# PersiaML/PERSIA

Hardware: AMD Instinct MI355X
Metric: samples/sec (whole node), DLRM-style hybrid training (higher is better)
Workload: dtype bf16; 1 GPU; preset=criteo, model=dlrm 26sparse/13dense dim128, global_batch=8192, rows=100000000, capacity_per_rank=100000000, staleness=8, parallelism=dp1+emb-a2a

## Files before the change

persia_amd/csrc/interact.hip:

```cpp
#include <torch/extension.h>
#include <ATen/hip/HIPContext.h>
#include <hip/hip_runtime.h>
#include <hip/hip_bf16.h>

namespace {

using bf16x8i = __attribute__((ext_vector_type(8))) short;
using bf16x4i = __attribute__((__vector_size__(4 * sizeof(__bf16)))) __bf16;
using f32x4i = __attribute__((ext_vector_type(4))) float;

__device__ __forceinline__ float ibf2f(short x) {
  union { float f; unsigned u; } v;
  v.u = ((unsigned)(unsigned short)x) << 16;
  return v.f;
}

__device__ __forceinline__ short if2bf(float f) {
  union { float f; unsigned u; } v;
  v.f = f;
  unsigned lsb = (v.u >> 16) & 1;
  v.u += 0x7fff + lsb;
  return (short)(v.u >> 16);
}

constexpr int ceil16(int x) { return (x + 15) & ~15; }
constexpr int ceil32(int x) { return (x + 31) & ~31; }

__global__ __launch_bounds__(256) void interact_fwd_mfma_kernel(
    const short* __restrict__ V, short* __restrict__ out, int B, int F, int D,
    int P) {
  extern __shared__ short lds[];
  const int waves = blockDim.x / 64;
  const int wave = threadIdx.x / 64, lane = threadIdx.x % 64;
  const int Fp = ceil16(F), Dk = ceil32(D);
  const int LDK = Dk + 8;
  const int T = Fp / 16;
  short* v = lds + wave * Fp * LDK;
  for (int t = lane; t < Fp * LDK / 8; t += 64) *(bf16x8i*)&v[t * 8] = bf16x8i{};
  const int fi = lane & 15;
  const int fk8 = (lane >> 4) * 8;
  const int d8 = D / 8;
  for (int64_t b = (int64_t)blockIdx.x * waves + wave; b < B;
       b += (int64_t)gridDim.x * waves) {
    const short* src = V + b * F * D;
    for (int t = lane; t < F * d8; t += 64) {
      const int fr = t / d8, c8 = (t % d8) * 8;
      *(bf16x8i*)&v[fr * LDK + c8] = *(const bf16x8i*)&src[fr * D + c8];
    }
    short* dst = out + b * P;
    for (int ti = 0; ti < T; ++ti) {
      for (int tj = 0; tj <= ti; ++tj) {
        f32x4i acc = {};
        for (int k = 0; k < Dk; k += 32) {
          const bf16x8i a = *(const bf16x8i*)&v[(ti * 16 + fi) * LDK + k + fk8];
          const bf16x8i c = *(const bf16x8i*)&v[(tj * 16 + fi) * LDK + k + fk8];
          acc = __builtin_amdgcn_mfma_f32_16x16x32_bf16(a, c, acc, 0, 0, 0);
        }
        const int j = tj * 16 + fi;
#pragma unroll
        for (int r = 0; r < 4; ++r) {
          const int i = ti * 16 + (lane >> 4) * 4 + r;
          if (i < F && j < i) dst[i * (i - 1) / 2 + j] = if2bf(acc[r]);
        }
      }
    }
  }
}

__global__ __launch_bounds__(256) void interact_bwd_mfma_kernel(
    const short* __restrict__ g, const short* __restrict__ V,
    short* __restrict__ dV, int B, int F, int D, int P) {
  extern __shared__ short lds[];
  const int waves = blockDim.x / 64;
  const int wave = threadIdx.x / 64, lane = threadIdx.x % 64;
  const int Fp = ceil16(F), Fk = ceil32(F), Dp = ceil16(D);
  const int LDA = Fk + 8;
  short* A = lds + wave * (Fp + Dp) * LDA;
  short* vt = A + Fp * LDA;
  for (int t = lane; t < (Fp + Dp) * LDA / 8; t += 64)
    *(bf16x8i*)&A[t * 8] = bf16x8i{};
  const int Tm = Fp / 16, Tn = Dp / 16;
  const int fi = lane & 15;
  const int fk8 = (lane >> 4) * 8;
  const int d8 = D / 8;
  for (int64_t b = (int64_t)blockIdx.x * waves + wave; b < B;
       b += (int64_t)gridDim.x * waves) {
    const short* src = V + b * F * D;
    for (int t = lane; t < F * d8; t += 64) {
      const int fr = t / d8, c8 = (t % d8) * 8;
      const bf16x8i row = *(const bf16x8i*)&src[fr * D + c8];
#pragma unroll
      for (int k = 0; k < 8; ++k) vt[(c8 + k) * LDA + fr] = row[k];
    }
    const short* gp = g + b * P;
    for (int p = lane; p < P; p += 64) {
      int i = (int)((1.0f + sqrtf(1.0f + 8.0f * (float)p)) * 0.5f);
      while (i * (i - 1) / 2 > p) --i;
      while ((i + 1) * i / 2 <= p) ++i;
      const int j = p - i * (i - 1) / 2;
      const short gv = gp[p];
      A[i * LDA + j] = gv;
      A[j * LDA + i] = gv;
    }
    short* dst = dV + b * F * D;
    for (int ti = 0; ti < Tm; ++ti) {
      for (int td = 0; td < Tn; ++td) {
        f32x4i acc = {};
        for (int k = 0; k < Fk; k += 32) {
          const bf16x8i a = *(const bf16x8i*)&A[(ti * 16 + fi) * LDA + k + fk8];
          const bf16x8i c = *(const bf16x8i*)&vt[(td * 16 + fi) * LDA + k + fk8];
          acc = __builtin_amdgcn_mfma_f32_16x16x32_bf16(a, c, acc, 0, 0, 0);
        }
        const int d = td * 16 + fi;
        if (d < D) {
#pragma unroll
          for (int r = 0; r < 4; ++r) {
            const int i = ti * 16 + (lane >> 4) * 4 + r;
            if (i < F) dst[i * D + d] = if2bf(acc[r]);
          }
        }
      }
    }
  }
}

__global__ __launch_bounds__(256) void interact_fwd_packed_kernel(
    const short* __restrict__ x, const __half* __restrict__ base,
    short* __restrict__ out, int B, int S, int D, int P) {
  extern __shared__ short lds[];
  const int F = S + 1;
  const int waves = blockDim.x / 64;
  const int wave = threadIdx.x / 64, lane = threadIdx.x % 64;
  const int Fp = ceil16(F), Dk = ceil32(D);
  const int LDK = Dk + 8;
  const int T = Fp / 16;
  short* v = lds + wave * Fp * LDK;
  for (int t = lane; t < Fp * LDK / 8; t += 64) *(bf16x8i*)&v[t * 8] = bf16x8i{};
  const int fi = lane & 15;
  const int fk8 = (lane >> 4) * 8;
  const int d8 = D / 8;
  for (int64_t b = (int64_t)blockIdx.x * waves + wave; b < B;
       b += (int64_t)gridDim.x * waves) {
    for (int t = lane; t < F * d8; t += 64) {
      const int fr = t / d8, c8 = (t % d8) * 8;
      bf16x8i val;
      if (fr == 0) {
        val = *(const bf16x8i*)&x[b * D + c8];
      } else {
        const __half* src = base + ((int64_t)(fr - 1) * B + b) * D + c8;
#pragma unroll
        for (int k = 0; k < 8; ++k) val[k] = if2bf(__half2float(src[k]));
      }
      *(bf16x8i*)&v[fr * LDK + c8] = val;
    }
    short* dst = out + b * P;
    for (int ti = 0; ti < T; ++ti) {
      for (int tj = 0; tj <= ti; ++tj) {
        f32x4i acc = {};
        for (int k = 0; k < Dk; k += 32) {
          const bf16x8i a = *(const bf16x8i*)&v[(ti * 16 + fi) * LDK + k + fk8];
          const bf16x8i c = *(const bf16x8i*)&v[(tj * 16 + fi) * LDK + k + fk8];
          acc = __builtin_amdgcn_mfma_f32_16x16x32_bf16(a, c, acc, 0, 0, 0);
        }
        const int j = tj * 16 + fi;
#pragma unroll
        for (int r = 0; r < 4; ++r) {
          const int i = ti * 16 + (lane >> 4) * 4 + r;
          if (i < F && j < i) dst[i * (i - 1) / 2 + j] = if2bf(acc[r]);
        }
      }
    }
  }
}

__global__ __launch_bounds__(256) void interact_bwd_packed_kernel(
    const short* __restrict__ g, const short* __restrict__ x,
    const __half* __restrict__ base, short* __restrict__ dx,
    __half* __restrict__ dbase, int B, int S, int D, int P) {
  extern __shared__ short lds[];
  const int F = S + 1;
  const int waves = blockDim.x / 64;
  const int wave = threadIdx.x / 64, lane = threadIdx.x % 64;
  const int Fp = ceil16(F), Fk = ceil32(F), Dp = ceil16(D);
  const int LDA = Fk + 8;
  const int LDV = Dp + 8;
  short* A = lds + wave * (Fp * LDA + Fk * LDV);
  short* v = A + Fp * LDA;
  for (int t = lane; t < (Fp * LDA + Fk * LDV) / 8; t += 64)
    *(bf16x8i*)&A[t * 8] = bf16x8i{};
  const int Tm = Fp / 16, Tn = Dp / 16;
  const int fi = lane & 15;
  const int fk8 = (lane >> 4) * 8;
  const int d8 = D / 8;
  const int t_ro = ((lane & 15) >> 2);
  const int t_co = (lane & 3) * 4;
  auto vtr = [&](int kb, int td) {
    const short* b0 = &v[(kb + fk8 + t_ro) * LDV + td * 16 + t_co];
    bf16x4i lo = __builtin_amdgcn_ds_read_tr16_b64_v4bf16(
        (__attribute__((address_space(3))) bf16x4i*)(void*)const_cast<short*>(b0));
    bf16x4i hi = __builtin_amdgcn_ds_read_tr16_b64_v4bf16(
        (__attribute__((address_space(3))) bf16x4i*)(void*)const_cast<short*>(b0 + 4 * LDV));
    bf16x8i r;
#pragma unroll
    for (int j = 0; j < 4; ++j) {
      r[j] = ((const short*)&lo)[j];
      r[4 + j] = ((const short*)&hi)[j];
    }
    return r;
  };
  for (int64_t b = (int64_t)blockIdx.x * waves + wave; b < B;
       b += (int64_t)gridDim.x * waves) {
    for (int t = lane; t < F * d8; t += 64) {
      const int fr = t / d8, c8 = (t % d8) * 8;
      bf16x8i row;
      if (fr == 0) {
        row = *(const bf16x8i*)&x[b * D + c8];
      } else {
        const __half* src = base + ((int64_t)(fr - 1) * B + b) * D + c8;
#pragma unroll
        for (int k = 0; k < 8; ++k) row[k] = if2bf(__half2float(src[k]));
      }
      *(bf16x8i*)&v[fr * LDV + c8] = row;
    }
    const short* gp = g + b * P;
    for (int p = lane; p < P; p += 64) {
      int i = (int)((1.0f + sqrtf(1.0f + 8.0f * (float)p)) * 0.5f);
      while (i * (i - 1) / 2 > p) --i;
      while ((i + 1) * i / 2 <= p) ++i;
      const int j = p - i * (i - 1) / 2;
      const short gv = gp[p];
      A[i * LDA + j] = gv;
      A[j * LDA + i] = gv;
    }
    for (int ti = 0; ti < Tm; ++ti) {
      for (int td = 0; td < Tn; ++td) {
        f32x4i acc = {};
        for (int k = 0; k < Fk; k += 32) {
          const bf16x8i a = *(const bf16x8i*)&A[(ti * 16 + fi) * LDA + k + fk8];
          const bf16x8i c = vtr(k, td);
          acc = __builtin_amdgcn_mfma_f32_16x16x32_bf16(a, c, acc, 0, 0, 0);
        }
        const int d = td * 16 + fi;
        if (d < D) {
#pragma unroll
          for (int r = 0; r < 4; ++r) {
            const int i = ti * 16 + (lane >> 4) * 4 + r;
            if (i == 0) {
              dx[b * D + d] = if2bf(acc[r]);
            } else if (i < F) {
              dbase[((int64_t)(i - 1) * B + b) * D + d] = __float2half(acc[r]);
            }
          }
        }
      }
    }
  }
}

__global__ __launch_bounds__(256) void interact_fwd_kernel(
    const short* __restrict__ V, short* __restrict__ out, int B, int F, int D,
    int P) {
  extern __shared__ short lds[];
  const int wave = threadIdx.x / 64, lane = threadIdx.x % 64;
  const int LD = D + 8;
  short* v = lds + wave * F * LD;
  const int64_t stride = (int64_t)gridDim.x * 4;
  const int64_t rounds = ((int64_t)B + stride - 1) / stride;
  for (int64_t r = 0; r < rounds; ++r) {
    const int64_t b = r * stride + (int64_t)blockIdx.x * 4 + wave;
    if (b < B) {
      const short* src = V + b * F * D;
      const int d8 = D / 8;
      for (int t = lane; t < F * d8; t += 64) {
        const int fr = t / d8, c8 = (t % d8) * 8;
        *(bf16x8i*)&v[fr * LD + c8] = *(const bf16x8i*)&src[fr * D + c8];
      }
    }
    __syncthreads();
    if (b < B) {
      for (int p = lane; p < P; p += 64) {
        int i = (int)((1.0f + sqrtf(1.0f + 8.0f * (float)p)) * 0.5f);
        while (i * (i - 1) / 2 > p) --i;
        while ((i + 1) * i / 2 <= p) ++i;
        const int j = p - i * (i - 1) / 2;
        const short* vi = &v[i * LD];
        const short* vj = &v[j * LD];
        float acc = 0.0f;
        for (int d = 0; d < D; d += 8) {
          bf16x8i a = *(const bf16x8i*)&vi[d];
          bf16x8i c = *(const bf16x8i*)&vj[d];
#pragma unroll
          for (int k = 0; k < 8; ++k) acc += ibf2f(a[k]) * ibf2f(c[k]);
        }
        out[b * P + p] = if2bf(acc);
      }
    }
    __syncthreads();
  }
}

__global__ __launch_bounds__(256) void interact_bwd_kernel(
    const short* __restrict__ g, const short* __restrict__ V,
    short* __restrict__ dV, int B, int F, int D, int P) {
  extern __shared__ short lds[];
  const int wave = threadIdx.x / 64, lane = threadIdx.x % 64;
  const int LD = D + 8;
  short* v = lds + wave * (F * LD + F * F);
  short* G = v + F * LD;
  const int64_t stride = (int64_t)gridDim.x * 4;
  const int64_t rounds = ((int64_t)B + stride - 1) / stride;
  for (int64_t r = 0; r < rounds; ++r) {
    const int64_t b = r * stride + (int64_t)blockIdx.x * 4 + wave;
    if (b < B) {
      const short* src = V + b * F * D;
      const int d8l = D / 8;
      for (int t = lane; t < F * d8l; t += 64) {
        const int fr = t / d8l, c8 = (t % d8l) * 8;
        *(bf16x8i*)&v[fr * LD + c8] = *(const bf16x8i*)&src[fr * D + c8];
      }
      for (int t = lane; t < F * F; t += 64) G[t] = 0;
    }
    __syncthreads();
    if (b < B) {
      const short* gp = g + b * P;
      for (int p = lane; p < P; p += 64) {
        int i = (int)((1.0f + sqrtf(1.0f + 8.0f * (float)p)) * 0.5f);
        while (i * (i - 1) / 2 > p) --i;
        while ((i + 1) * i / 2 <= p) ++i;
        const int j = p - i * (i - 1) / 2;
        const short gv = gp[p];
        G[i * F + j] = gv;
        G[j * F + i] = gv;
      }
    }
    __syncthreads();
    if (b < B) {
      const int d8 = D / 8;
      short* dst = dV + b * F * D;
      for (int t = lane; t < F * d8; t += 64) {
        const int i = t / d8, dd = (t % d8) * 8;
        float acc[8] = {};
        for (int j = 0; j < F; ++j) {
          const float gij = ibf2f(G[i * F + j]);
          if (gij != 0.0f) {
            const short* vj = &v[j * LD + dd];
#pragma unroll
            for (int k = 0; k < 8; ++k) acc[k] += gij * ibf2f(vj[k]);
          }
        }
#pragma unroll
        for (int k = 0; k < 8; ++k) dst[i * D + dd + k] = if2bf(acc[k]);
      }
    }
    __syncthreads();
  }
}

inline int pick_waves(int per_wave_shorts) {
  const int bytes = per_wave_shorts * 2;
  for (int w = 4; w >= 1; w >>= 1)
    if (w * bytes <= 65536) return w;
  return 0;
}

}

static hipStream_t icur_stream() {
  return at::hip::getCurrentHIPStream().stream();
}

torch::Tensor interact_fwd(torch::Tensor V) {
  TORCH_CHECK(V.scalar_type() == torch::kBFloat16 && V.is_contiguous());
  const int B = (int)V.size(0), F = (int)V.size(1), D = (int)V.size(2);
  TORCH_CHECK(D % 8 == 0);
  const int P = F * (F - 1) / 2;
  auto out = torch::empty(
      {B, P}, torch::TensorOptions().dtype(torch::kBFloat16).device(V.device()));
  const int Fp = ceil16(F), Dk = ceil32(D);
  const int mfma_shorts = Fp * (Dk + 8);
  const int waves = pick_waves(mfma_shorts);
  if (waves > 0) {
    const int grid = std::min((B + waves - 1) / waves, 8192);
    hipLaunchKernelGGL(interact_fwd_mfma_kernel, dim3(grid),
                       dim3(waves * 64), waves * mfma_shorts * 2,
                       icur_stream(), (const short*)V.data_ptr(),
                       (short*)out.data_ptr(), B, F, D, P);
    return out;
  }
  const int lds = 4 * F * (D + 8) * 2;
  TORCH_CHECK(lds <= 65536, "interaction tile exceeds LDS");
  const int grid = std::min((B + 3) / 4, 8192);
  hipLaunchKernelGGL(interact_fwd_kernel, dim3(grid), dim3(256), lds,
                     icur_stream(), (const short*)V.data_ptr(),
                     (short*)out.data_ptr(), B, F, D, P);
  return out;
}

torch::Tensor interact_bwd(torch::Tensor g, torch::Tensor V) {
  const int B = (int)V.size(0), F = (int)V.size(1), D = (int)V.size(2);
  const int P = F * (F - 1) / 2;
  auto dV = torch::empty_like(V);
  const int Fp = ceil16(F), Fk = ceil32(F), Dp = ceil16(D);
  const int mfma_shorts = (Fp + Dp) * (Fk + 8);
  const int waves = pick_waves(mfma_shorts);
  if (waves > 0) {
    const int grid = std::min((B + waves - 1) / waves, 8192);
    hipLaunchKernelGGL(interact_bwd_mfma_kernel, dim3(grid),
                       dim3(waves * 64), waves * mfma_shorts * 2,
                       icur_stream(), (const short*)g.data_ptr(),
                       (const short*)V.data_ptr(), (short*)dV.data_ptr(), B, F,
                       D, P);
    return dV;
  }
  const int lds = 4 * (F * (D + 8) * 2 + 2 * F * F);
  TORCH_CHECK(lds <= 65536, "interaction tile exceeds LDS");
  const int grid = std::min((B + 3) / 4, 8192);
  hipLaunchKernelGGL(interact_bwd_kernel, dim3(grid), dim3(256), lds,
                     icur_stream(), (const short*)g.data_ptr(),
                     (const short*)V.data_ptr(), (short*)dV.data_ptr(), B, F,
                     D, P);
  return dV;
}

torch::Tensor interact_fwd_packed(torch::Tensor x, torch::Tensor base) {
  TORCH_CHECK(x.scalar_type() == torch::kBFloat16 && x.is_contiguous());
  TORCH_CHECK(base.scalar_type() == torch::kFloat16 && base.is_contiguous());
  const int B = (int)x.size(0), D = (int)x.size(1);
  const int S = (int)(base.size(0) / B);
  const int F = S + 1;
  TORCH_CHECK(D % 8 == 0 && base.size(1) == D && base.size(0) == (int64_t)S * B);
  const int P = F * (F - 1) / 2;
  auto out = torch::empty(
      {B, P}, torch::TensorOptions().dtype(torch::kBFloat16).device(x.device()));
  const int Fp = ceil16(F), Dk = ceil32(D);
  const int mfma_shorts = Fp * (Dk + 8);
  const int waves = pick_waves(mfma_shorts);
  TORCH_CHECK(waves > 0, "interact_fwd_packed: tile exceeds LDS");
  const int grid = std::min((B + waves - 1) / waves, 8192);
  hipLaunchKernelGGL(interact_fwd_packed_kernel, dim3(grid), dim3(waves * 64),
                     waves * mfma_shorts * 2, icur_stream(),
                     (const short*)x.data_ptr(),
                     (const __half*)base.data_ptr<at::Half>(),
                     (short*)out.data_ptr(), B, S, D, P);
  return out;
}

std::vector<torch::Tensor> interact_bwd_packed(torch::Tensor g, torch::Tensor x,
                                               torch::Tensor base) {
  const int B = (int)x.size(0), D = (int)x.size(1);
  const int S = (int)(base.size(0) / B);
  const int F = S + 1;
  const int P = F * (F - 1) / 2;
  auto dx = torch::empty_like(x);
  auto dbase = torch::empty_like(base);
  const int Fp = ceil16(F), Fk = ceil32(F), Dp = ceil16(D);
  const int mfma_shorts = Fp * (Fk + 8) + Fk * (Dp + 8);
  const int waves = pick_waves(mfma_shorts);
  TORCH_CHECK(waves > 0, "interact_bwd_packed: tile exceeds LDS");
  const int grid = std::min((B + waves - 1) / waves, 8192);
  auto gc = g.contiguous();
  hipLaunchKernelGGL(interact_bwd_packed_kernel, dim3(grid), dim3(waves * 64),
                     waves * mfma_shorts * 2, icur_stream(),
                     (const short*)gc.data_ptr(),
                     (const short*)x.data_ptr(),
                     (const __half*)base.data_ptr<at::Half>(),
                     (short*)dx.data_ptr(), (__half*)dbase.data_ptr<at::Half>(),
                     B, S, D, P);
  return {dx, dbase};
}

bool interact_packed_feasible(int64_t F, int64_t D) {
  if (D % 8 != 0) return false;
  const int Fp = ceil16((int)F), Fk = ceil32((int)F), Dp = ceil16((int)D),
            Dk = ceil32((int)D);
  return pick_waves(Fp * (Dk + 8)) > 0 &&
         pick_waves(Fp * (Fk + 8) + Fk * (Dp + 8)) > 0;
}

bool interact_feasible(int64_t F, int64_t D) {
  if (D % 8 != 0) return false;
  const int Fp = ceil16((int)F), Fk = ceil32((int)F), Dp = ceil16((int)D),
            Dk = ceil32((int)D);
  const bool fwd_ok = pick_waves(Fp * (Dk + 8)) > 0 ||
                      4 * (int)F * ((int)D + 8) * 2 <= 65536;
  const bool bwd_ok =
      pick_waves((Fp + Dp) * (Fk + 8)) > 0 ||
      4 * ((int)F * ((int)D + 8) * 2 + 2 * (int)F * (int)F) <= 65536;
  return fwd_ok && bwd_ok;
}

void init_interact(pybind11::module_& m) {
  m.def("interact_fwd", &interact_fwd, "DLRM pairwise dot interaction");
  m.def("interact_bwd", &interact_bwd, "interaction backward (dV)");
  m.def("interact_feasible", &interact_feasible,
        "true if a fused interaction kernel exists for (F, D)");
  m.def("interact_packed_feasible", &interact_packed_feasible,
        "true if the packed-input MFMA interaction fits (F, D)");
  m.def("interact_fwd_packed", &interact_fwd_packed,
        "interaction from (x bf16 [B,D], slot-major f16 base) directly");
  m.def("interact_bwd_packed", &interact_bwd_packed,
        "packed interaction backward -> (dx, dbase f16)");
}
```

persia_amd/models/dlrm.py:

```python
from typing import List

import torch
import torch.nn as nn


class _BlasLinearFn(torch.autograd.Function):

    @staticmethod
    def forward(ctx, x, w, b):
        ctx.save_for_backward(x, w)
        return torch.nn.functional.linear(x, w, b)

    @staticmethod
    def backward(ctx, g):
        from persia_amd.ops import native

        x, w = ctx.saved_tensors
        g = g.contiguous()
        dx = g @ w
        dw = g.t() @ x
        db = native().bias_grad(g).to(w.dtype)
        return dx, dw, db


class PALinear(nn.Linear):

    def forward(self, x):
        import os

        if (
            x.is_cuda and x.dim() == 2 and self.bias is not None
            and x.dtype == self.weight.dtype and x.dtype == torch.bfloat16
            and os.environ.get("PA_BLAS_LINEAR", "0") == "1"
        ):
            from persia_amd.ops import native_available

            if native_available():
                return _BlasLinearFn.apply(x, self.weight, self.bias)
        return super().forward(x)


def _mlp(sizes: List[int], last_relu: bool = False) -> nn.Sequential:
    layers: List[nn.Module] = []
    for i in range(len(sizes) - 1):
        layers.append(PALinear(sizes[i], sizes[i + 1]))
        if i < len(sizes) - 2 or last_relu:
            layers.append(nn.ReLU())
    return nn.Sequential(*layers)


class _InteractFn(torch.autograd.Function):

    @staticmethod
    def forward(ctx, v):
        from persia_amd.ops import native

        v = v.to(torch.bfloat16).contiguous()
        ctx.save_for_backward(v)
        return native().interact_fwd(v)

    @staticmethod
    def backward(ctx, g):
        from persia_amd.ops import native

        (v,) = ctx.saved_tensors
        return native().interact_bwd(g.to(torch.bfloat16).contiguous(), v)


class _InteractPackedFn(torch.autograd.Function):

    @staticmethod
    def forward(ctx, x, base):
        from persia_amd.ops import native

        x = x.contiguous()
        base = base.contiguous()
        ctx.save_for_backward(x, base)
        return native().interact_fwd_packed(x, base)

    @staticmethod
    def backward(ctx, g):
        from persia_amd.ops import native

        x, base = ctx.saved_tensors
        dx, dbase = native().interact_bwd_packed(g, x, base)
        return dx, dbase


class DotInteraction(nn.Module):

    def forward(self, vectors: torch.Tensor) -> torch.Tensor:
        F, D = vectors.shape[1], vectors.shape[2]
        if vectors.is_cuda and D % 8 == 0:
            from persia_amd.ops import native, native_available

            if native_available() and native().interact_feasible(F, D):
                return _InteractFn.apply(vectors)
        B, F, _D = vectors.shape
        prod = torch.bmm(vectors, vectors.transpose(1, 2))
        li, lj = torch.tril_indices(F, F, offset=-1, device=vectors.device)
        return prod[:, li, lj]


class DLRM(nn.Module):
    def __init__(
        self,
        num_sparse: int = 26,
        num_dense: int = 13,
        dim: int = 128,
        bottom_mlp: List[int] = (512, 256, 128),
        top_mlp: List[int] = (1024, 1024, 512, 256),
        fused: bool = False,
    ):
        super().__init__()
        self.dim = dim
        self.num_sparse = num_sparse
        n_f = num_sparse + 1
        inter_out = n_f * (n_f - 1) // 2
        if fused:
            from persia_amd.ops.dense import FusedMLP

            self.bottom = FusedMLP([num_dense] + list(bottom_mlp) + [dim], last_relu=True)
            self.top = FusedMLP([dim + inter_out] + list(top_mlp) + [1])
        else:
            self.bottom = _mlp([num_dense] + list(bottom_mlp) + [dim], last_relu=True)
            self.top = _mlp([dim + inter_out] + list(top_mlp) + [1])
        self.interaction = DotInteraction()

    def forward(
        self, non_id_tensors, embedding_tensors
    ) -> torch.Tensor:
        dense = (
            non_id_tensors if torch.is_tensor(non_id_tensors) else non_id_tensors[0]
        )
        dt = next(self.bottom.parameters()).dtype
        dense = dense.to(dt)
        x = self.bottom(dense)
        if torch.is_tensor(embedding_tensors):
            B = x.shape[0]
            if (
                x.is_cuda
                and x.dtype == torch.bfloat16
                and embedding_tensors.dtype == torch.float16
                and self.dim % 8 == 0
            ):
                from persia_amd.ops import native, native_available

                if native_available() and native().interact_packed_feasible(
                    self.num_sparse + 1, self.dim
                ):
                    inter = _InteractPackedFn.apply(x, embedding_tensors)
                    k = x.shape[1] + inter.shape[1]
                    pad = (-k) % 128
                    parts = [x, inter]
                    if pad:
                        parts.append(x.new_zeros(B, pad))
                    return self.top(torch.cat(parts, dim=1)).squeeze(1)
            emb = (
                embedding_tensors.view(self.num_sparse, B, self.dim)
                .permute(1, 0, 2)
                .to(x.dtype)
            )
            vectors = torch.cat([x.unsqueeze(1), emb], dim=1)
        else:
            vectors = torch.stack([x] + [e.to(x.dtype) for e in embedding_tensors], dim=1)
        inter = self.interaction(vectors)
        out = self.top(torch.cat([x, inter], dim=1))
        return out.squeeze(1)
```

Baseline: 7.854 million samples/s.

## Fuse interaction output concat/pad and backward grad slicing into packed kernels

Forward now writes x, the pairwise dot products and the zero padding directly into the padded top-MLP input buffer, which removes the separate torch.cat and zero-fill. A new backward kernel reads the full top-input gradient with a stride, adds the dx slice in-kernel, and can accumulate the embedding gradient in place into base.grad. It also uses vectorized f16->bf16 conversion and the LDS transpose-read instruction (ds_read_tr16) for the dV matmul. This cuts extra elementwise kernels and memory traffic, at the cost of more kernel complexity and a sqrt-based pair index decode per element.

```diff
diff --git a/persia_amd/csrc/interact.hip b/persia_amd/csrc/interact.hip
--- a/persia_amd/csrc/interact.hip
+++ b/persia_amd/csrc/interact.hip
@@ -124,9 +124,10 @@
   }
 }
 
+template <bool INTO>
 __global__ __launch_bounds__(256) void interact_fwd_packed_kernel(
     const short* __restrict__ x, const __half* __restrict__ base,
-    short* __restrict__ out, int B, int S, int D, int P) {
+    short* __restrict__ out, int B, int S, int D, int P, int ldo) {
   extern __shared__ short lds[];
   const int F = S + 1;
   const int waves = blockDim.x / 64;
@@ -146,6 +147,7 @@
       bf16x8i val;
       if (fr == 0) {
         val = *(const bf16x8i*)&x[b * D + c8];
+        if (INTO) *(bf16x8i*)&out[b * ldo + c8] = val;
       } else {
         const __half* src = base + ((int64_t)(fr - 1) * B + b) * D + c8;
 #pragma unroll
@@ -153,7 +155,9 @@
       }
       *(bf16x8i*)&v[fr * LDK + c8] = val;
     }
-    short* dst = out + b * P;
+    short* dst = out + b * ldo + (INTO ? D : 0);
+    if (INTO)
+      for (int t = P + lane; t < ldo - D; t += 64) dst[t] = 0;
     for (int ti = 0; ti < T; ++ti) {
       for (int tj = 0; tj <= ti; ++tj) {
         f32x4i acc = {};
@@ -257,6 +261,179 @@
   }
 }
 
+__device__ __forceinline__ void wave_lds_fence() {
+  asm volatile("s_waitcnt lgkmcnt(0)" ::: "memory");
+  __builtin_amdgcn_wave_barrier();
+}
+
+__device__ __forceinline__ short if2bf_nan(float f) {
+  return f != f ? (short)0x7fc0 : if2bf(f);
+}
+
+using f16x8 = __attribute__((ext_vector_type(8))) _Float16;
+using f16x4 = __attribute__((ext_vector_type(4))) _Float16;
+using f32x8 = __attribute__((ext_vector_type(8))) float;
+using hbf16x8 = __attribute__((ext_vector_type(8))) __bf16;
+using hbf16x4 = __attribute__((ext_vector_type(4))) __bf16;
+using s16x4 = __attribute__((ext_vector_type(4))) short;
+
+__device__ __forceinline__ bf16x8i f16x8_to_bf16(f16x8 h) {
+  const hbf16x8 r =
+      __builtin_convertvector(__builtin_convertvector(h, f32x8), hbf16x8);
+  return __builtin_bit_cast(bf16x8i, r);
+}
+
+struct ChunkWalk {
+  int fr, c;
+  __device__ __forceinline__ void next(int q64, int r64, int d8) {
+    fr += q64;
+    c += r64;
+    if (c >= d8) {
+      c -= d8;
+      ++fr;
+    }
+  }
+};
+
+template <int NK>
+__global__ __launch_bounds__(256) void interact_bwd_packed_io_kernel(
+    const short* __restrict__ g, int ldg, int gcol,
+    const short* __restrict__ x, const __half* __restrict__ base,
+    const short* __restrict__ gx, short* __restrict__ dx, short* dbase,
+    int accumulate, int B, int S, int D, int P) {
+  extern __shared__ short lds[];
+  const int F = S + 1;
+  const int waves = blockDim.x / 64;
+  const int wave = threadIdx.x / 64, lane = threadIdx.x % 64;
+  constexpr int Fk = NK * 32;
+  const int Fp = ceil16(F), Dp = ceil16(D);
+  const int LDA = Fk + 8;
+  const int LDV = Dp + 8;
+  short* A = lds + wave * (Fp * LDA + Fk * LDV);
+  short* v = A + Fp * LDA;
+  for (int t = lane; t < (Fp * LDA + Fk * LDV) / 8; t += 64)
+    *(bf16x8i*)&A[t * 8] = bf16x8i{};
+  const int Tm = Fp / 16, Tn = Dp / 16;
+  const int fi = lane & 15;
+  const int fk8 = (lane >> 4) * 8;
+  const int d8 = D / 8;
+  const int n8 = F * d8;
+  const int t_ro = ((lane & 15) >> 2);
+  const int t_co = (lane & 3) * 4;
+  auto vtr = [&](int kb, int td) {
+    const short* b0 = &v[(kb + fk8 + t_ro) * LDV + td * 16 + t_co];
+    bf16x4i lo = __builtin_amdgcn_ds_read_tr16_b64_v4bf16(
+        (__attribute__((address_space(3))) bf16x4i*)(void*)const_cast<short*>(b0));
+    bf16x4i hi = __builtin_amdgcn_ds_read_tr16_b64_v4bf16(
+        (__attribute__((address_space(3))) bf16x4i*)(void*)const_cast<short*>(b0 + 4 * LDV));
+    bf16x8i r;
+#pragma unroll
+    for (int j = 0; j < 4; ++j) {
+      r[j] = ((const short*)&lo)[j];
+      r[4 + j] = ((const short*)&hi)[j];
+    }
+    return r;
+  };
+  const ChunkWalk w0 = {lane / d8, lane % d8};
+  const int q64 = 64 / d8, r64 = 64 % d8;
+  wave_lds_fence();
+  for (int64_t b = (int64_t)blockIdx.x * waves + wave; b < B;
+       b += (int64_t)gridDim.x * waves) {
+    ChunkWalk w = w0;
+    for (int t = lane; t < n8; t += 64, w.next(q64, r64, d8)) {
+      const int fr = w.fr, c8 = w.c * 8;
+      bf16x8i row;
+      if (fr == 0) {
+        row = *(const bf16x8i*)&x[b * D + c8];
+      } else {
+        row = f16x8_to_bf16(
+            *(const f16x8*)(base + ((int64_t)(fr - 1) * B + b) * D + c8));
+      }
+      *(bf16x8i*)&v[fr * LDV + c8] = row;
+    }
+    const short* gp = g + b * ldg + gcol;
+    for (int p = lane; p < P; p += 64) {
+      int i = (int)((1.0f + sqrtf(1.0f + 8.0f * (float)p)) * 0.5f);
+      while (i * (i - 1) / 2 > p) --i;
+      while ((i + 1) * i / 2 <= p) ++i;
+      const int j = p - i * (i - 1) / 2;
+      const short gv = gp[p];
+      A[i * LDA + j] = gv;
+      A[j * LDA + i] = gv;
+    }
+    wave_lds_fence();
+    for (int td = 0; td < Tn; ++td) {
+      bf16x8i c[NK];
+#pragma unroll
+      for (int kk = 0; kk < NK; ++kk) c[kk] = vtr(kk * 32, td);
+      wave_lds_fence();
+      const int d0 = td * 16 + (lane >> 4) * 4;
+      for (int ti = 0; ti < Tm; ++ti) {
+        f32x4i acc = {};
+#pragma unroll
+        for (int kk = 0; kk < NK; ++kk) {
+          const bf16x8i a =
+              *(const bf16x8i*)&A[(ti * 16 + fi) * LDA + kk * 32 + fk8];
+          acc = __builtin_amdgcn_mfma_f32_16x16x32_bf16(c[kk], a, acc, 0, 0, 0);
+        }
+        const int i = ti * 16 + fi;
+        if (i < F && d0 < D) {
+          const s16x4 as_bf16 = __builtin_bit_cast(
+              s16x4, __builtin_convertvector(acc, hbf16x4));
+          const s16x4 as_f16 = __builtin_bit_cast(
+              s16x4, __builtin_convertvector(acc, f16x4));
+          *(s16x4*)&v[i * LDV + d0] = i == 0 ? as_bf16 : as_f16;
+        }
+      }
+    }
+    wave_lds_fence();
+    w = w0;
+    for (int t0 = 0; t0 < n8; t0 += 4 * 64) {
+      bf16x8i o[4], old[4];
+      int frs[4], c8s[4];
+#pragma unroll
+      for (int u = 0; u < 4; ++u) {
+        const int t = t0 + u * 64 + lane;
+        frs[u] = w.fr;
+        c8s[u] = w.c * 8;
+        w.next(q64, r64, d8);
+        if (t < n8) {
+          const int fr = frs[u], c8 = c8s[u];
+          o[u] = *(const bf16x8i*)&v[fr * LDV + c8];
+          if (fr == 0) {
+            if (gx) old[u] = *(const bf16x8i*)&gx[b * ldg + c8];
+          } else if (accumulate) {
+            old[u] = *(const bf16x8i*)&dbase[((int64_t)(fr - 1) * B + b) * D + c8];
+          }
+        }
+      }
+#pragma unroll
+      for (int u = 0; u < 4; ++u) {
+        const int t = t0 + u * 64 + lane;
+        if (t < n8) {
+          const int fr = frs[u], c8 = c8s[u];
+          bf16x8i res = o[u];
+          if (fr == 0) {
+            if (gx) {
+#pragma unroll
+              for (int k = 0; k < 8; ++k)
+                res[k] = if2bf_nan(ibf2f(old[u][k]) + ibf2f(o[u][k]));
+            }
+            *(bf16x8i*)&dx[b * D + c8] = res;
+          } else {
+            if (accumulate)
+              res = __builtin_bit_cast(
+                  bf16x8i, __builtin_bit_cast(f16x8, old[u]) +
+                               __builtin_bit_cast(f16x8, o[u]));
+            *(bf16x8i*)&dbase[((int64_t)(fr - 1) * B + b) * D + c8] = res;
+          }
+        }
+      }
+    }
+    wave_lds_fence();
+  }
+}
+
 __global__ __launch_bounds__(256) void interact_fwd_kernel(
     const short* __restrict__ V, short* __restrict__ out, int B, int F, int D,
     int P) {
@@ -422,7 +599,10 @@
   return dV;
 }
 
-torch::Tensor interact_fwd_packed(torch::Tensor x, torch::Tensor base) {
+static torch::Tensor interact_fwd_packed_impl(torch::Tensor x,
+                                              torch::Tensor base, int64_t Kp) {
+  TORCH_CHECK(x.is_cuda() && base.is_cuda() && x.device() == base.device());
+  TORCH_CHECK(x.dim() == 2 && base.dim() == 2 && x.size(0) > 0);
   TORCH_CHECK(x.scalar_type() == torch::kBFloat16 && x.is_contiguous());
   TORCH_CHECK(base.scalar_type() == torch::kFloat16 && base.is_contiguous());
   const int B = (int)x.size(0), D = (int)x.size(1);
@@ -430,19 +610,35 @@
   const int F = S + 1;
   TORCH_CHECK(D % 8 == 0 && base.size(1) == D && base.size(0) == (int64_t)S * B);
   const int P = F * (F - 1) / 2;
+  const bool into = Kp >= 0;
+  TORCH_CHECK(!into || (Kp >= D + P && Kp % 8 == 0),
+              "interact_fwd_packed_into: Kp must be a multiple of 8 and >= D + P");
   auto out = torch::empty(
-      {B, P}, torch::TensorOptions().dtype(torch::kBFloat16).device(x.device()));
+      {B, into ? Kp : (int64_t)P},
+      torch::TensorOptions().dtype(torch::kBFloat16).device(x.device()));
   const int Fp = ceil16(F), Dk = ceil32(D);
   const int mfma_shorts = Fp * (Dk + 8);
   const int waves = pick_waves(mfma_shorts);
   TORCH_CHECK(waves > 0, "interact_fwd_packed: tile exceeds LDS");
   const int grid = std::min((B + waves - 1) / waves, 8192);
-  hipLaunchKernelGGL(interact_fwd_packed_kernel, dim3(grid), dim3(waves * 64),
+  auto kernel = into ? interact_fwd_packed_kernel<true>
+                     : interact_fwd_packed_kernel<false>;
+  hipLaunchKernelGGL(kernel, dim3(grid), dim3(waves * 64),
                      waves * mfma_shorts * 2, icur_stream(),
                      (const short*)x.data_ptr(),
                      (const __half*)base.data_ptr<at::Half>(),
-                     (short*)out.data_ptr(), B, S, D, P);
+                     (short*)out.data_ptr(), B, S, D, P, (int)out.size(1));
   return out;
+}
+
+torch::Tensor interact_fwd_packed(torch::Tensor x, torch::Tensor base) {
+  return interact_fwd_packed_impl(x, base, -1);
+}
+
+torch::Tensor interact_fwd_packed_into(torch::Tensor x, torch::Tensor base,
+                                       int64_t Kp) {
+  TORCH_CHECK(Kp >= 0, "interact_fwd_packed_into: negative Kp");
+  return interact_fwd_packed_impl(x, base, Kp);
 }
 
 std::vector<torch::Tensor> interact_bwd_packed(torch::Tensor g, torch::Tensor x,
@@ -469,6 +665,70 @@
   return {dx, dbase};
 }
 
+static bool aligned16(const torch::Tensor& t) {
+  return reinterpret_cast<uintptr_t>(t.data_ptr()) % 16 == 0;
+}
+
+std::vector<torch::Tensor> interact_bwd_packed_acc(
+    torch::Tensor g, torch::Tensor x, torch::Tensor base,
+    c10::optional<torch::Tensor> grad) {
+  TORCH_CHECK(g.is_cuda() && x.device() == g.device() &&
+              base.device() == g.device());
+  TORCH_CHECK(g.dim() == 2 && x.dim() == 2 && base.dim() == 2 && x.size(0) > 0);
+  TORCH_CHECK(g.scalar_type() == torch::kBFloat16 &&
+              x.scalar_type() == torch::kBFloat16 && x.is_contiguous());
+  TORCH_CHECK(base.scalar_type() == torch::kFloat16 && base.is_contiguous());
+  const int B = (int)x.size(0), D = (int)x.size(1);
+  const int S = (int)(base.size(0) / B);
+  const int F = S + 1;
+  TORCH_CHECK(D % 8 == 0 && base.size(1) == D && base.size(0) == (int64_t)S * B);
+  const int P = F * (F - 1) / 2;
+  TORCH_CHECK(g.size(0) == B && g.size(1) >= D + P,
+              "interact_bwd_packed_acc: g must be [B, Kp] with Kp >= D + P");
+  TORCH_CHECK(g.size(1) == 1 || g.stride(1) == 1);
+  TORCH_CHECK(g.stride(0) >= g.size(1) && g.stride(0) < (1 << 30));
+  const bool acc = grad.has_value() && grad->defined();
+  if (acc)
+    TORCH_CHECK(grad->scalar_type() == torch::kFloat16 &&
+                    grad->is_contiguous() && grad->sizes() == base.sizes() &&
+                    grad->device() == base.device(),
+                "interact_bwd_packed_acc: grad must match base (f16, contiguous)");
+  const int Fp = ceil16(F), Fk = ceil32(F), Dp = ceil16(D);
+  const int mfma_shorts = Fp * (Fk + 8) + Fk * (Dp + 8);
+  const int waves = pick_waves(mfma_shorts);
+  TORCH_CHECK(waves > 0, "interact_bwd_packed_acc: tile exceeds LDS");
+  const int NK = Fk / 32;
+  if (NK > 5 || !aligned16(g) || g.stride(0) % 8 != 0 || !aligned16(x) ||
+      !aligned16(base) || (acc && !aligned16(*grad))) {
+    auto r = interact_bwd_packed(g.narrow(1, D, P), x, base);
+    auto dx = g.narrow(1, 0, D) + r[0];
+    if (!acc) return {dx, r[1]};
+    grad->add_(r[1]);
+    return {dx};
+  }
+  auto dx = torch::empty_like(x);
+  auto dbase = acc ? *grad : torch::empty_like(base);
+  const int grid = std::min((B + waves - 1) / waves, 8192);
+  auto launch = [&](auto kernel) {
+    hipLaunchKernelGGL(kernel, dim3(grid), dim3(waves * 64),
+                       waves * mfma_shorts * 2, icur_stream(),
+                       (const short*)g.data_ptr(), (int)g.stride(0), D,
+                       (const short*)x.data_ptr(),
+                       (const __half*)base.data_ptr<at::Half>(),
+                       (const short*)g.data_ptr(), (short*)dx.data_ptr(),
+                       (short*)dbase.data_ptr(), acc ? 1 : 0, B, S, D, P);
+  };
+  switch (NK) {
+    case 1: launch(interact_bwd_packed_io_kernel<1>); break;
+    case 2: launch(interact_bwd_packed_io_kernel<2>); break;
+    case 3: launch(interact_bwd_packed_io_kernel<3>); break;
+    case 4: launch(interact_bwd_packed_io_kernel<4>); break;
+    default: launch(interact_bwd_packed_io_kernel<5>); break;
+  }
+  if (acc) return {dx};
+  return {dx, dbase};
+}
+
 bool interact_packed_feasible(int64_t F, int64_t D) {
   if (D % 8 != 0) return false;
   const int Fp = ceil16((int)F), Fk = ceil32((int)F), Dp = ceil16((int)D),
@@ -500,4 +760,11 @@
         "interaction from (x bf16 [B,D], slot-major f16 base) directly");
   m.def("interact_bwd_packed", &interact_bwd_packed,
         "packed interaction backward -> (dx, dbase f16)");
-}
+  m.def("interact_fwd_packed_into", &interact_fwd_packed_into,
+        "packed interaction forward -> [B, Kp] = [x | pairs | zeros]");
+  m.def("interact_bwd_packed_acc", &interact_bwd_packed_acc,
+        "backward of interact_fwd_packed_into from g [B, Kp]; adds the "
+        "embedding gradient into `grad` in place when given -> (dx[, dbase])",
+        pybind11::arg("g"), pybind11::arg("x"), pybind11::arg("base"),
+        pybind11::arg("grad") = pybind11::none());
+}
diff --git a/persia_amd/models/dlrm.py b/persia_amd/models/dlrm.py
--- a/persia_amd/models/dlrm.py
+++ b/persia_amd/models/dlrm.py
@@ -67,7 +67,7 @@
         return native().interact_bwd(g.to(torch.bfloat16).contiguous(), v)
 
 
-class _InteractPackedFn(torch.autograd.Function):
+class _InteractPackedPairsFn(torch.autograd.Function):
 
     @staticmethod
     def forward(ctx, x, base):
@@ -85,6 +85,66 @@
         x, base = ctx.saved_tensors
         dx, dbase = native().interact_bwd_packed(g, x, base)
         return dx, dbase
+
+
+def _grad_accumulable(base: torch.Tensor) -> bool:
+    if not (base.is_leaf and base.requires_grad):
+        return False
+    g = base.grad
+    return (
+        g is not None
+        and g.dtype == torch.float16
+        and g.is_contiguous()
+        and g.shape == base.shape
+        and g.device == base.device
+        and not torch.is_grad_enabled()
+        and not base._backward_hooks
+        and not getattr(base, "_post_accumulate_grad_hooks", None)
+    )
+
+
+class _InteractPackedFn(torch.autograd.Function):
+
+    @staticmethod
+    def forward(ctx, x, base):
+        from persia_amd.ops import native
+
+        x = x.contiguous()
+        base = base.contiguous()
+        ctx.save_for_backward(x, base)
+        n_f = base.shape[0] // x.shape[0] + 1
+        k = x.shape[1] + n_f * (n_f - 1) // 2
+        return native().interact_fwd_packed_into(x, base, (k + 127) // 128 * 128)
+
+    @staticmethod
+    def backward(ctx, g):
+        from persia_amd.ops import native
+
+        x, base = ctx.saved_tensors
+        if g.stride(-1) != 1:
+            g = g.contiguous()
+        if ctx.needs_input_grad[1] and _grad_accumulable(base):
+            (dx,) = native().interact_bwd_packed_acc(g, x, base, base.grad)
+            return dx, None
+        dx, dbase = native().interact_bwd_packed_acc(g, x, base, None)
+        return dx, dbase
+
+
+def _fused_interact_io() -> bool:
+    import os
+
+    return os.environ.get("PA_INTERACT_FUSED_IO", "1") != "0"
+
+
+def packed_top_input(x: torch.Tensor, base: torch.Tensor) -> torch.Tensor:
+    if _fused_interact_io():
+        return _InteractPackedFn.apply(x, base)
+    inter = _InteractPackedPairsFn.apply(x, base)
+    pad = (-(x.shape[1] + inter.shape[1])) % 128
+    parts = [x, inter]
+    if pad:
+        parts.append(x.new_zeros(x.shape[0], pad))
+    return torch.cat(parts, dim=1)
 
 
 class DotInteraction(nn.Module):
@@ -149,13 +209,9 @@
                 if native_available() and native().interact_packed_feasible(
                     self.num_sparse + 1, self.dim
                 ):
-                    inter = _InteractPackedFn.apply(x, embedding_tensors)
-                    k = x.shape[1] + inter.shape[1]
-                    pad = (-k) % 128
-                    parts = [x, inter]
-                    if pad:
-                        parts.append(x.new_zeros(B, pad))
-                    return self.top(torch.cat(parts, dim=1)).squeeze(1)
+                    return self.top(
+                        packed_top_input(x, embedding_tensors)
+                    ).squeeze(1)
             emb = (
                 embedding_tensors.view(self.num_sparse, B, self.dim)
                 .permute(1, 0, 2)
```

New measurement: 7.973 million samples/s (median of 6 runs). +1.5%, better.
